# IsseiMori/lajolla_public

Hardware: AMD Instinct MI355X
Metric: Msamples/sec (whole node), cbox 256spp (higher is better)
Workload: dtype f32; 1 GPU; cbox.xml 512x512 @ 256 spp, path integrator (Lambertian + area light, max_depth -1, rr_depth 5); rng=pcg32, one stream per (pixel, sample), seed 0x853c49e6748fea9b, parallelism=1 GPU, collective=none

## Files before the change

### lajolla_public_amd/csrc/device/api_device.hip

```cpp
#include "api_internal.h"

namespace {

void set_device(lj_context *ctx) { HIP_CHECK(hipSetDevice(ctx->device)); }

ljd::DQueue carve_queue(void *base, uint32_t cap) {
    ljd::DQueue q{};
    ljd::Rec4 *p = (ljd::Rec4 *)base;
    auto take = [&]() { ljd::Rec4 *r = p; p += cap; return r; };
    q.ro = take(); q.rd = take(); q.rs = take(); q.rh = take(); q.rw = take(); q.rl = take(); q.rn = take(); q.rg = take();
    return q;
}
size_t queue_bytes(uint32_t cap) { return (size_t)cap * kQueueSlotBytes; }

void ensure_queues(lj_context *ctx, uint32_t cap) {
    if (ctx->queue_capacity >= cap) return;
    cap = (cap + 63u) & ~63u;
    ctx->queue_mem.alloc(queue_bytes(cap));
    ctx->queue_capacity = cap;
}

int *ensure_spill(lj_context *ctx, int levels, uint32_t grid) {
    if (levels <= 0) return nullptr;
    const size_t need = (size_t)levels * grid * 256 * sizeof(int);
// ... 142 lines not shown
    }
    if (plan.rng_mode == LJ_RNG_TILE) { run_tiles(sc, plan, ds, rgb_dev, samples_host, stream); return; }
    const uint64_t max_samples_pass = (uint64_t)1 << 27;
    uint64_t pix_per_pass = std::max<uint64_t>(1, max_samples_pass / (uint64_t)plan.spp);
    pix_per_pass = std::min<uint64_t>(pix_per_pass, n_pix);
    if (sc->flat.integrator == LJ_INTEGRATOR_VOLPATH) {
        const uint64_t pass_samples_max = pix_per_pass * (uint64_t)plan.spp;
        if (ctx->sample_rgb.bytes < pass_samples_max * 12) ctx->sample_rgb.alloc(pass_samples_max * 12);
        if (!ctx->chunk_counter.p) ctx->chunk_counter.alloc(128 * kMaxLanes);
        upload_pixel_list(ctx, plan, stream);
        HIP_CHECK(hipMemsetAsync(ctx->chunk_counter.p, 0, 256, stream));
        HIP_CHECK(hipEventRecord(ctx->ev_begin, stream));
        for (uint64_t p0 = 0; p0 < n_pix; p0 += pix_per_pass) {
            const uint64_t np = std::min<uint64_t>(pix_per_pass, n_pix - p0);
            const uint64_t total = np * (uint64_t)plan.spp;
            ljd::DPass pass{};
            pass.pixel_list = (const uint32_t *)ctx->pixel_list.p + p0; pass.n_pixels = (uint32_t)np; ljd::set_pass_divisors(pass, (uint32_t)plan.spp, (uint32_t)sc->flat.cam.width);
            pass.seed = plan.seed; pass.sample_rgb = (float *)ctx->sample_rgb.p;
            const int grid = (int)std::max<uint64_t>(1, std::min<uint64_t>((total + 255) / 256, (uint64_t)ctx->n_cus * (uint64_t)ljd::volpath_blocks_per_cu(ds)));
            HIP_CHECK(hipMemsetAsync((char *)ctx->chunk_counter.p + 8, 0, 4, stream));
            ljd::launch_volpath(ds, pass, (uint32_t)total, (uint32_t *)ctx->chunk_counter.p, sc->ecfg, sc->scfg.variant,
                                 (sc->feat_kinds & ~7u) == 0u && !sc->feat_textured && !sc->feat_envmap && !sc->feat_sphere_lights,
                                ensure_spill(ctx, sc->ecfg.spill_levels, (uint32_t)grid), grid, stream);
            HIP_CHECK(hipGetLastError());
            st.samples += total; st.wavefront_steps++;
            if (rgb_dev) ljd::launch_resolve(pass, (uint32_t)np, rgb_dev, stream);
            if (samples_host) {
                HIP_CHECK(hipMemcpyAsync(samples_host + p0 * (uint64_t)plan.spp * 3, ctx->sample_rgb.p, total * 12, hipMemcpyDeviceToHost, stream));
                HIP_CHECK(hipStreamSynchronize(stream));
            }
        }
        HIP_CHECK(hipEventRecord(ctx->ev_end, stream));
        HIP_CHECK(hipEventSynchronize(ctx->ev_end));
        float ms = 0; HIP_CHECK(hipEventElapsedTime(&ms, ctx->ev_begin, ctx->ev_end));
        unsigned long long nb = 0;
        HIP_CHECK(hipMemcpy(&nb, ctx->chunk_counter.p, 8, hipMemcpyDeviceToHost));
        st.render_ms = ms; st.bounce_iterations = nb;
        if (getenv("LJ_VOLPATH_STATS")) {
            unsigned long long h[32];
            HIP_CHECK(hipMemcpy(h, ctx->chunk_counter.p, sizeof(h), hipMemcpyDeviceToHost));
            const char *names[8] = {"node iterations", "leaf steps", "closest calls", "tracking (bounce ray)", "tracking (shadow segment)", "shadow segments", "path steps", "-"};
            for (int k = 0; k < 7; k++) fprintf(stderr, "[volpath stats] %-26s wave events %12llu  lanes active %5.1f %%  per sample %.2f\n", names[k], h[2 + 2 * k], h[2 + 2 * k] ? 100.0 * h[3 + 2 * k] / (64.0 * h[2 + 2 * k]) : 0.0, (double)h[3 + 2 * k] / (double)st.samples);
        }
        return;
    }
    const size_t mega_lds = ljd::mega_smem(sc->dscene, sc->scfg);
    const bool mega_off = getenv("LJ_TUNE_MEGA") && atoi(getenv("LJ_TUNE_MEGA")) == 0;
    if (mega_lds > 0 && !mega_off) {
        const uint64_t pass_samples_max = pix_per_pass * (uint64_t)plan.spp;
        if (ctx->sample_rgb.bytes < pass_samples_max * 12) ctx->sample_rgb.alloc(pass_samples_max * 12);
        if (!ctx->mega_state.p) ctx->mega_state.alloc(64);
        upload_pixel_list(ctx, plan, stream);
        HIP_CHECK(hipEventRecord(ctx->ev_begin, stream));
        int per_cu = ljd::mega_blocks_per_cu(sc->scfg);
        if (const char *e = getenv("LJ_TUNE_MEGA_BLOCKS_PER_CU")) per_cu = std::max(1, atoi(e));
        uint32_t grab_max = 768, grab_min = 192;
        bool grab_fixed = false;
        if (const char *e = getenv("LJ_TUNE_MEGA_GRAB")) { grab_max = (uint32_t)std::max(64, atoi(e)) & ~63u; grab_fixed = true; }
        double mega_ms = 0;
        unsigned long long hstats[5] = {};
        for (uint64_t p0 = 0; p0 < n_pix; p0 += pix_per_pass) {
            const uint64_t np = std::min<uint64_t>(pix_per_pass, n_pix - p0);
            const uint64_t total = np * (uint64_t)plan.spp;
            ljd::DPass pass{};
            pass.pixel_list = (const uint32_t *)ctx->pixel_list.p + p0; pass.n_pixels = (uint32_t)np; ljd::set_pass_divisors(pass, (uint32_t)plan.spp, (uint32_t)sc->flat.cam.width);
            pass.seed = plan.seed; pass.sample_rgb = (float *)ctx->sample_rgb.p;
            HIP_CHECK(hipMemsetAsync(ctx->mega_state.p, 0, 64, stream));
            uint32_t grab = grab_max;
            if (!grab_fixed) {
                uint64_t draws = 16;
                if (const char *e = getenv("LJ_TUNE_MEGA_DRAWS")) draws = (uint64_t)std::max(1, atoi(e));
                const uint64_t waves = (uint64_t)ctx->n_cus * per_cu * 4, per_draw = total / (waves * draws);
                grab = (uint32_t)std::min<uint64_t>(grab_max, std::max<uint64_t>(grab_min, per_draw & ~(uint64_t)63));
            }
            const uint64_t pieces = (total + grab - 1) / grab;
            const int grid = (int)std::max<uint64_t>(1, std::min<uint64_t>((uint64_t)ctx->n_cus * per_cu, (pieces + 3) / 4));
            if (timing) HIP_CHECK(hipEventRecord(ctx->ev_k0, stream));
            ljd::launch_mega(ds, pass, sc->scfg, sc->flat.n_spheres > 0, (uint32_t)total, grab, (uint32_t *)ctx->mega_state.p,
                             (unsigned long long *)((char *)ctx->mega_state.p + 8), grid, stream);
            HIP_CHECK(hipGetLastError());
            if (timing) {
                HIP_CHECK(hipEventRecord(ctx->ev_k1, stream)); HIP_CHECK(hipEventSynchronize(ctx->ev_k1));
                float a = 0; HIP_CHECK(hipEventElapsedTime(&a, ctx->ev_k0, ctx->ev_k1)); mega_ms += a;
            }
            st.mega_launches++; st.wavefront_steps++;
            if (rgb_dev) ljd::launch_resolve(pass, (uint32_t)np, rgb_dev, stream);
            unsigned long long *h = ctx->stats_host;
            HIP_CHECK(hipMemcpyAsync(h, (char *)ctx->mega_state.p + 8, 5 * sizeof(unsigned long long), hipMemcpyDeviceToHost, stream));
            if (samples_host) HIP_CHECK(hipMemcpyAsync(samples_host + p0 * (uint64_t)plan.spp * 3, ctx->sample_rgb.p, total * 12, hipMemcpyDeviceToHost, stream));
            HIP_CHECK(hipStreamSynchronize(stream));
            if (h[3] != total)
                throw LjError(LJ_ERR_INTERNAL, "mega launch ended with " + std::to_string(h[3]) + " of " + std::to_string(total) + " samples finished");
            for (int k = 0; k < 5; k++) hstats[k] += h[k];
            st.samples += total;
        }
        HIP_CHECK(hipEventRecord(ctx->ev_end, stream));
        HIP_CHECK(hipEventSynchronize(ctx->ev_end));
        float ms = 0; HIP_CHECK(hipEventElapsedTime(&ms, ctx->ev_begin, ctx->ev_end));
        st.render_ms = ms; st.mega_ms = mega_ms;
        st.bounce_iterations = hstats[0]; st.rays_closest = hstats[1]; st.rays_shadow = hstats[2]; st.path_steps = hstats[4];
        st.mega_bytes = st.samples * 12ull + n_pix * 4ull;
        st.queue_bytes = st.mega_bytes;
        return;
    }
    const uint64_t pass_samples_max = pix_per_pass * (uint64_t)plan.spp;
    uint32_t pool = (uint32_t)std::min<uint64_t>(plan.pool, std::max<uint64_t>(pass_samples_max, 256));
    uint32_t blocks_per_cu = 8;
    if (const char *e = getenv("LJ_TUNE_BLOCKS_PER_CU")) blocks_per_cu = (uint32_t)std::max(1, atoi(e));
    unsigned long long *xstats = nullptr;
    DevBuf xstats_buf;
    if (getenv("LJ_EXTEND_STATS")) { xstats_buf.alloc(64); HIP_CHECK(hipMemsetAsync(xstats_buf.p, 0, 64, stream)); xstats = (unsigned long long *)xstats_buf.p; }
    uint32_t n_lanes = (timing || xstats || pool < (1u << 20)) ? 1u : (pool < (1u << 22) ? 2u : 4u);
    if (sc->scfg.variant >= 4) n_lanes = 1;
    const bool large_tree = ds.n_nodes > sc->ecfg.lds_nodes;
    if (large_tree) n_lanes = 1;
    if (const char *e = getenv("LJ_TUNE_LANES")) n_lanes = (uint32_t)std::min((int)kMaxLanes, std::max(1, atoi(e)));
    uint32_t n_blocks = std::min<uint32_t>(kMaxBlocks, std::max<uint32_t>(n_lanes, std::min<uint32_t>((uint32_t)ctx->n_cus * blocks_per_cu, pool / 256)));
    n_blocks = (n_blocks / n_lanes) * n_lanes;
    const uint32_t lane_blocks = n_blocks / n_lanes;
    uint32_t seg = ((pool + n_blocks - 1) / n_blocks + 255u) & ~255u;
    const uint32_t n_slots = n_blocks * seg, lane_slots = lane_blocks * seg;
    ensure_queues(ctx, n_slots);
    const bool sort_segments = ljd::shade_sorts_segments(sc->scfg);
    if (sort_segments) {
        const uint32_t cap = (n_slots + 63u) & ~63u;
        if (ctx->queue2_capacity < cap) { ctx->queue_mem2.alloc(queue_bytes(cap)); ctx->queue2_capacity = cap; }
        if (ctx->sort_perm.bytes < (size_t)cap * 4) ctx->sort_perm.alloc((size_t)cap * 4);
        if (ctx->sort_keys.bytes < (size_t)cap) ctx->sort_keys.alloc((size_t)cap);
    }
    uint32_t ext_per_cu = n_lanes == 1 ? 8 : (n_lanes == 2 ? 4 : 2);
    if (const char *e = getenv("LJ_TUNE_EXTEND_BLOCKS_PER_CU")) ext_per_cu = (uint32_t)std::max(1, atoi(e));
    const uint32_t lane_chunks = lane_slots / 256u;
    const uint32_t ext_grid = std::max<uint32_t>(1, std::min<uint32_t>((uint32_t)ctx->n_cus * ext_per_cu, (lane_chunks + 3) / 4));
    bool use_tail = !timing && !xstats && !large_tree && ljd::tail_smem(sc->ecfg, sc->scfg) > 0;
    if (const char *e = getenv("LJ_TUNE_TAIL")) use_tail = use_tail && atoi(e) != 0;
    uint64_t tail_num = 1, tail_den = 4;
    if (const char *e = getenv("LJ_TUNE_TAIL_FRAC")) { tail_num = (uint64_t)std::max(1, atoi(e)); tail_den = 16; }
    const uint32_t spill_grid = std::max<uint32_t>(ext_grid, use_tail ? lane_blocks : 0u);
    int *spill_base = ensure_spill(ctx, sc->ecfg.spill_levels, spill_grid * n_lanes);
    if (!ctx->chunk_counter.p) ctx->chunk_counter.alloc(128 * kMaxLanes);
    if (ctx->chunk_list.bytes < (size_t)lane_chunks * 8 * n_lanes) ctx->chunk_list.alloc((size_t)lane_chunks * 8 * n_lanes);
    const ljd::DQueue q_all = carve_queue(ctx->queue_mem.p, ctx->queue_capacity);
    const ljd::DQueue q2_all = sort_segments ? carve_queue(ctx->queue_mem2.p, ctx->queue2_capacity) : q_all;
    struct Lane {
        hipStream_t stream; ljd::DQueue q, q2; uint32_t *sort_perm; uint8_t *sort_keys; ljd::DBlockState *dblocks; ljd::DBlockState *hblocks;
        uint32_t *work; uint32_t *lists[2]; uint32_t parity; int *spill; int *spill_tail; bool done; int batch;
    } lanes[kMaxLanes];
    for (uint32_t l = 0; l < n_lanes; l++) {
        Lane &L = lanes[l];
        L.stream = l == 0 ? stream : ctx->lane_streams[l - 1];
        const size_t o = (size_t)l * lane_slots;
        L.q = q_all; L.q.ro += o; L.q.rd += o; L.q.rs += o; L.q.rh += o; L.q.rw += o; L.q.rl += o; L.q.rn += o; L.q.rg += o;
// ... 86 lines not shown
            }
            if (!any) break;
        }
        uint64_t samples_done = 0, path_steps = 0, shadow_rays = 0;
        for (uint32_t b = 0; b < n_blocks; b++) {
            const ljd::DBlockState &bs = ctx->blocks_host[b];
            samples_done += bs.samples_done; path_steps += bs.path_steps; shadow_rays += bs.rays_shadow;
            st.bounce_iterations += bs.bounce_iterations; st.rays_closest += bs.rays_closest; st.rays_shadow += bs.rays_shadow;
        }
        if (samples_done != total)
            throw LjError(LJ_ERR_INTERNAL, "wavefront loop ended with " + std::to_string(samples_done) + " of " + std::to_string(total) + " samples finished");
        st.samples += total;
        st.path_steps += path_steps;
        st.extend_bytes += path_steps * 48ull + shadow_rays * 16ull;
        st.shade_bytes += path_steps * 224ull + total * 12ull;
        if (rgb_dev) ljd::launch_resolve(pass, (uint32_t)np, rgb_dev, stream);
        if (samples_host) {
            HIP_CHECK(hipMemcpyAsync(samples_host + p0 * (uint64_t)plan.spp * 3, ctx->sample_rgb.p, total * 12, hipMemcpyDeviceToHost, stream));
            HIP_CHECK(hipStreamSynchronize(stream));
        }
    }
    HIP_CHECK(hipEventRecord(ctx->ev_end, stream));
    HIP_CHECK(hipEventSynchronize(ctx->ev_end));
    float ms = 0; HIP_CHECK(hipEventElapsedTime(&ms, ctx->ev_begin, ctx->ev_end));
    st.render_ms = ms; st.extend_ms = extend_ms; st.shade_ms = shade_ms;
    if (xstats) {
        unsigned long long h[8];
        HIP_CHECK(hipMemcpy(h, xstats, 64, hipMemcpyDeviceToHost));
        fprintf(stderr, "[extend stats] rays %llu | outer iters %llu busy lanes %.1f%% | node steps %llu (%.2f/ray) lane use %.1f%% | prim rounds %llu (%.2f tests/ray) lane use %.1f%% | refills %llu\n",
                h[7], h[0], 100.0 * h[1] / (64.0 * h[0]), h[2], (double)h[3] / h[7], 100.0 * h[3] / (64.0 * h[2]), h[4], (double)h[5] / h[7], 100.0 * h[5] / (64.0 * h[4]), h[6]);
    }
    st.queue_bytes = st.extend_bytes + st.shade_bytes;
}

}

extern "C" {

int lj_context_create(int device_id, lj_context **out) {
    return lj::guard([&]() {
        if (!out) throw LjError(LJ_ERR_INVALID_ARG, "lj_context_create: null out");
        *out = nullptr;
        int n = 0;
        hipError_t e = hipGetDeviceCount(&n);
        if (e != hipSuccess || n == 0) throw LjError(LJ_ERR_DEVICE, std::string("no HIP device available (") + hipGetErrorString(e) + "); this library has no CPU path");
        if (device_id < 0 || device_id >= n) throw LjError(LJ_ERR_INVALID_ARG, "device id out of range");
        auto ctx = std::make_unique<lj_context>();
        ctx->device = device_id;
        HIP_CHECK(hipSetDevice(device_id));
        hipDeviceProp_t prop; HIP_CHECK(hipGetDeviceProperties(&prop, device_id));
        if (std::string(prop.gcnArchName).rfind("gfx950", 0) != 0)
            throw LjError(LJ_ERR_DEVICE, std::string("device is ") + prop.gcnArchName + "; this build contains gfx950 code objects only");
        ctx->n_cus = prop.multiProcessorCount;
        HIP_CHECK(hipStreamCreateWithFlags(&ctx->stream, hipStreamNonBlocking));
        for (auto &ls : ctx->lane_streams) HIP_CHECK(hipStreamCreateWithFlags(&ls, hipStreamNonBlocking));
        HIP_CHECK(hipEventCreateWithFlags(&ctx->ev_fork, hipEventDisableTiming)); HIP_CHECK(hipEventCreateWithFlags(&ctx->ev_join, hipEventDisableTiming));
        HIP_CHECK(hipEventCreateWithFlags(&ctx->ev_caller, hipEventDisableTiming));
        ctx->blocks.alloc(sizeof(ljd::DBlockState) * kMaxBlocks);
        HIP_CHECK(hipHostMalloc((void **)&ctx->blocks_host, sizeof(ljd::DBlockState) * kMaxBlocks, hipHostMallocDefault));
        HIP_CHECK(hipHostMalloc((void **)&ctx->stats_host, 64, hipHostMallocDefault));
        HIP_CHECK(hipEventCreate(&ctx->ev_begin)); HIP_CHECK(hipEventCreate(&ctx->ev_end));
        HIP_CHECK(hipEventCreate(&ctx->ev_k0)); HIP_CHECK(hipEventCreate(&ctx->ev_k1));
        *out = ctx.release();
    });
}

void lj_context_destroy(lj_context *ctx) {
    if (!ctx) return;
    if (ctx->live_scenes > 0) { ctx->doomed = true; return; }
    (void)hipSetDevice(ctx->device);
    if (ctx->stream) { (void)hipStreamSynchronize(ctx->stream); (void)hipStreamDestroy(ctx->stream); }
    for (auto &ls : ctx->lane_streams) if (ls) { (void)hipStreamSynchronize(ls); (void)hipStreamDestroy(ls); }
    if (ctx->ev_fork) (void)hipEventDestroy(ctx->ev_fork);
    if (ctx->ev_join) (void)hipEventDestroy(ctx->ev_join);
    if (ctx->ev_caller) (void)hipEventDestroy(ctx->ev_caller);
    if (ctx->blocks_host) (void)hipHostFree(ctx->blocks_host);
    if (ctx->stats_host) (void)hipHostFree(ctx->stats_host);
    for (hipEvent_t e : {ctx->ev_begin, ctx->ev_end, ctx->ev_k0, ctx->ev_k1}) if (e) (void)hipEventDestroy(e);
    delete ctx;
}

int lj_scene_upload(lj_context *ctx, const LjSceneDesc *desc, lj_scene **out) {
    return lj::guard([&]() {
        if (!ctx || !desc || !out) throw LjError(LJ_ERR_INVALID_ARG, "lj_scene_upload: null argument");
        *out = nullptr;
        set_device(ctx);
        auto sc = std::make_unique<lj_scene>();
        sc->ctx = ctx;
        sc->flat = lj::flatten_scene(*desc);
        lj::FlatScene &F = sc->flat;
        hipStream_t s = ctx->stream;
        upload(sc->nodes, F.nodes, s);
        int node8_stride = (int)sizeof(ljd::DNode8);
        if (const char *e = getenv("LJ_TUNE_NODE8_STRIDE")) node8_stride = atoi(e) >= 128 ? 128 : 80;
        std::vector<unsigned char> nodes8_padded;
        if (node8_stride == (int)sizeof(ljd::DNode8)) upload(sc->nodes8, F.nodes8, s);
        else {
            nodes8_padded.assign(F.nodes8.size() * (size_t)node8_stride, 0);
            for (size_t i = 0; i < F.nodes8.size(); i++) memcpy(&nodes8_padded[i * (size_t)node8_stride], &F.nodes8[i], sizeof(ljd::DNode8));
            upload(sc->nodes8, nodes8_padded, s);
        }
        upload(sc->leaf_prims, F.leaf_prims, s); upload(sc->prims, F.prims, s); upload(sc->spheres, F.spheres, s);
        upload(sc->materials, F.materials, s); upload(sc->lights, F.lights, s); upload(sc->light_cdf, F.light_cdf, s);
        upload(sc->light_tris, F.light_tris, s); upload(sc->light_tri_cdf, F.light_tri_cdf, s);
        upload(sc->images3, F.images3, s); upload(sc->images1, F.images1, s); upload(sc->texels, F.texels, s); upload(sc->env_tables, F.env_tables, s);
        upload(sc->media, F.media, s); upload(sc->volume_data, F.volume_data, s); upload(sc->shape_media, F.shape_media, s);
// ... 137 lines not shown
```

### lajolla_public_amd/csrc/device/api_internal.h

```cpp
#pragma once
#include <hip/hip_runtime.h>
#include "../host/api_common.h"
#include "../host/flatten.h"
#include "dtypes.h"
#include "dconfig.h"
#include <algorithm>
#include <cstdlib>
#include <cstring>
#include <memory>
#include <string>
#include <vector>

namespace ljd {
ShadeConfig shade_config(size_t n_prims, size_t n_materials, size_t n_lights, size_t n_light_tris, size_t n_light_tri_cdf, size_t n_images3, size_t n_images1, size_t n_env_marg);
int shade_variant(uint32_t kinds, bool textured, bool envmap, bool sphere_lights);
ExtendConfig extend_config(int n_nodes, int n_prims, int bvh_depth, int n_spheres, int n_nodes8, int bvh8_depth, bool open_scene);
int max_stack_depth();
void launch_extend(const DScene &sc, const DQueue &q, const DBlockState *blocks, uint32_t grid, uint32_t seg, uint32_t *work, const uint32_t *chunk_list, uint32_t parity, const ExtendConfig &cfg, int *spill, unsigned long long *stats, hipStream_t s);
bool shade_sorts_segments(const ShadeConfig &cfg);
void launch_shade(const DScene &sc, const DPass &pass, const DQueue &q, const DQueue &qo, uint32_t *sort_perm, uint8_t *sort_keys, DBlockState *blocks, uint32_t n_blocks, uint32_t seg, const ShadeConfig &cfg, uint32_t *work, uint32_t *chunk_list, uint32_t parity, uint32_t extend_waves, hipStream_t s);
void launch_resolve(const DPass &pass, uint32_t n_pixels, float *rgb, hipStream_t s);
size_t tail_smem(const ExtendConfig &ecfg, const ShadeConfig &scfg);
void launch_tail(const DScene &sc, const DPass &pass, const DQueue &q, DBlockState *blocks, uint32_t n_blocks, uint32_t seg, const ExtendConfig &ecfg, const ShadeConfig &scfg, int *spill, hipStream_t s);
void launch_aux(const DScene &sc, const uint32_t *pixel_list, uint32_t n_pixels, int integrator, float *rgb, const ExtendConfig &cfg, int *spill, int grid, hipStream_t s);
void launch_volpath(const DScene &sc, const DPass &pass, uint32_t n_samples, uint32_t *counters, const ExtendConfig &cfg, int shade_variant, bool plain, int *spill, int grid, hipStream_t s);
int volpath_blocks_per_cu(const DScene &sc);
void launch_trace_rays(const DScene &sc, const void *rays, long long n, void *hits, unsigned char *occ, const ExtendConfig &cfg, int *spill, int grid, hipStream_t s);
size_t mega_smem(const DScene &sc, const ShadeConfig &scfg);
int mega_blocks_per_cu(const ShadeConfig &scfg);
void launch_mega(const DScene &sc, const DPass &pass, const ShadeConfig &scfg, bool spheres, uint32_t n_samples, uint32_t grab, uint32_t *sample_counter, unsigned long long *stats, int grid, hipStream_t s);
void launch_trace_rays_scan(const DScene &sc, const void *rays, long long n, void *hits, unsigned char *occ, int grid, hipStream_t s);
size_t tile_cursor_bytes(bool vol);
void launch_tile_init(bool vol, void *cursors, const uint32_t *tiles, uint32_t n_tiles, uint64_t seed, hipStream_t s);
int tile_grid(uint32_t n_tiles, uint32_t lanes);
void launch_tile(bool vol, const DScene &sc, const DTileJob &job, void *cursors, uint32_t lanes, uint32_t budget, uint32_t *alive, const ExtendConfig &cfg, int *spill, hipStream_t s);
void tile_cursor_stats(bool vol, const void *cursors_host, uint32_t n, unsigned long long out[5]);
}

using lj::LjError;

#define HIP_CHECK(expr) do { hipError_t _e = (expr); if (_e != hipSuccess) \
    throw LjError(LJ_ERR_DEVICE, std::string(#expr) + " failed: " + hipGetErrorString(_e)); } while (0)

struct DevBuf {
    void *p = nullptr; size_t bytes = 0;
    void alloc(size_t n) { release(); if (n) { HIP_CHECK(hipMalloc(&p, n)); bytes = n; } }
    void release() { if (p) { (void)hipFree(p); p = nullptr; bytes = 0; } }
    ~DevBuf() { release(); }
    DevBuf() = default; DevBuf(const DevBuf &) = delete; DevBuf &operator=(const DevBuf &) = delete;
};

template <typename T> inline void upload(DevBuf &b, const std::vector<T> &v, hipStream_t s) {
    b.alloc(((std::max<size_t>(v.size(), 1) * sizeof(T)) + 31) & ~(size_t)15);
    if (!v.empty()) HIP_CHECK(hipMemcpyAsync(b.p, v.data(), v.size() * sizeof(T), hipMemcpyHostToDevice, s));
}

static constexpr size_t kQueueSlotBytes = 128;
static constexpr uint32_t kMaxBlocks = 8192;

static constexpr uint32_t kMaxLanes = 8;
struct lj_context {
    int device = 0;
    int live_scenes = 0; bool doomed = false;
    hipStream_t stream = nullptr;
    hipStream_t lane_streams[kMaxLanes - 1] = {};
    hipEvent_t ev_fork = nullptr, ev_join = nullptr, ev_caller = nullptr;
    int n_cus = 256;
    DevBuf queue_mem; uint32_t queue_capacity = 0;
    DevBuf queue_mem2, sort_perm, sort_keys; uint32_t queue2_capacity = 0;
    DevBuf chunk_counter, chunk_list;
    DevBuf spill;
    DevBuf blocks, sample_rgb, pixel_list, frame;
    uint64_t pixel_list_key = 0;
    DevBuf tile_cursors, tile_list, tile_samples;
    DevBuf mega_state;
    ljd::DBlockState *blocks_host = nullptr;
    unsigned long long *stats_host = nullptr;
    hipEvent_t ev_begin = nullptr, ev_end = nullptr, ev_k0 = nullptr, ev_k1 = nullptr;
};

struct lj_scene {
    lj_context *ctx = nullptr;
    lj::FlatScene flat;
    DevBuf nodes, nodes8, leaf_prims, prims, spheres, materials, lights, light_cdf, light_tris, light_tri_cdf, images3, images1, texels, env_tables;
    DevBuf media, volume_data, shape_media, scan_leaves;
    ljd::DScene dscene{};
    ljd::ExtendConfig ecfg{};
    ljd::ShadeConfig scfg{};
    uint32_t feat_kinds = 0; bool feat_textured = false, feat_envmap = false, feat_sphere_lights = false;
    std::shared_ptr<const std::vector<uint32_t>> plan_pixels; uint64_t plan_pixels_key = 0;
    std::vector<int64_t> shape_first_gprim;
    LjStats stats{};
};
```

### lajolla_public_amd/csrc/device/mega.hip

```cpp
#include "dstage.h"
#include "dtrace.h"
#include "dconfig.h"

namespace ljd {

#define LJ_CONST __attribute__((address_space(4)))

constexpr uint32_t kItemCap = 512;
constexpr uint32_t kWaveScanBytes = 64 * 48 + 64 * 8 + 64 * 4 + kItemCap * 2;

struct ScanCtx {
    const LJ_CONST float *boxes;
    int n_used;
    const LJ_LDS int *leaf_tab;
    const LJ_LDS v4f *lprims; int prim_stride;
    const DSphere *spheres;
    LJ_LDS v4f *rays;
    LJ_LDS unsigned long long *keys;
    LJ_LDS uint32_t *occl;
    LJ_LDS uint16_t *items;
};

__device__ __forceinline__ uint32_t lane_id() { return __builtin_amdgcn_mbcnt_hi(~0u, __builtin_amdgcn_mbcnt_lo(~0u, 0u)); }

struct ScanRay { float ix, iy, iz, ox, oy, oz; };
__device__ __forceinline__ ScanRay scan_ray(f3 org, f3 dir) {
    const float tiny = 1e-18f;
    const float dx = fabsf(dir.x) < tiny ? copysignf(tiny, dir.x) : dir.x, dy = fabsf(dir.y) < tiny ? copysignf(tiny, dir.y) : dir.y,
                dz = fabsf(dir.z) < tiny ? copysignf(tiny, dir.z) : dir.z;
    ScanRay r;
    r.ix = __builtin_amdgcn_rcpf(dx); r.iy = __builtin_amdgcn_rcpf(dy); r.iz = __builtin_amdgcn_rcpf(dz);
    r.ox = org.x * r.ix; r.oy = org.y * r.iy; r.oz = org.z * r.iz;
    return r;
}
template <bool FAR>
__device__ __forceinline__ float scan_box(const float (&b)[6], const ScanRay &r, float tnear, float tfar) {
    const float ax = __builtin_fmaf(b[0], r.ix, -r.ox), bx = __builtin_fmaf(b[3], r.ix, -r.ox);
    const float ay = __builtin_fmaf(b[1], r.iy, -r.oy), by = __builtin_fmaf(b[4], r.iy, -r.oy);
    const float az = __builtin_fmaf(b[2], r.iz, -r.oz), bz = __builtin_fmaf(b[5], r.iz, -r.oz);
    const float te = fmaxf(fmaxf(fminf(ax, bx), fminf(ay, by)), fmaxf(fminf(az, bz), tnear));
    float tx = fminf(fminf(fmaxf(ax, bx), fmaxf(ay, by)), fmaxf(az, bz));
    if (FAR) tx = fminf(tx, tfar);
    return __builtin_fmaf(tx, -1.0000005f, te);
}
__device__ __forceinline__ uint32_t shift_in_sign(uint32_t mask, float d) { return __builtin_amdgcn_alignbit(mask, f2u(d), 31u); }

template <bool E, bool S>
__device__ __forceinline__ void scan_leaf_boxes(const ScanCtx &sx, const ScanRay &re, float tnear_e, const ScanRay &rs, float tnear_s, float tfar_s, uint32_t &me, uint32_t &ms) {
    const int n = sx.n_used;
    int k = 0;
    for (; k + 4 <= n; k += 4) {
        float b[4][6];
#pragma unroll
        for (int c = 0; c < 4; c++)
#pragma unroll
            for (int j = 0; j < 6; j++) b[c][j] = sx.boxes[(k + c) * 8 + j];
#pragma unroll
        for (int c = 0; c < 4; c++) {
            if (E) me = shift_in_sign(me, scan_box<false>(b[c], re, tnear_e, INFINITY));
            if (S) ms = shift_in_sign(ms, scan_box<true>(b[c], rs, tnear_s, tfar_s));
        }
    }
    for (; k < n; k++) {
        float b[6];
#pragma unroll
        for (int j = 0; j < 6; j++) b[j] = sx.boxes[k * 8 + j];
        if (E) me = shift_in_sign(me, scan_box<false>(b, re, tnear_e, INFINITY));
        if (S) ms = shift_in_sign(ms, scan_box<true>(b, rs, tnear_s, tfar_s));
    }
}
__device__ __forceinline__ void scan_leaf_boxes2(const ScanCtx &sx, f3 org, f3 dir_e, float tnear_e, f3 dir_s, float tnear_s, float tfar_s, bool any_e, bool any_s,
                                                 uint32_t &me, uint32_t &ms) {
    const ScanRay re = scan_ray(org, dir_e), rs = scan_ray(org, dir_s);
    tnear_e = fmaxf(tnear_e, 0.0f); tnear_s = fmaxf(tnear_s, 0.0f);
    me = 0u; ms = 0u;
    if (any_e && any_s) scan_leaf_boxes<true, true>(sx, re, tnear_e, rs, tnear_s, tfar_s, me, ms);
    else if (any_e) scan_leaf_boxes<true, false>(sx, re, tnear_e, rs, tnear_s, tfar_s, me, ms);
    else if (any_s) scan_leaf_boxes<false, true>(sx, re, tnear_e, rs, tnear_s, tfar_s, me, ms);
}

template <bool SPHERES>
__device__ __forceinline__ void scan_trace(const ScanCtx &sx, bool has_e, bool has_s, f3 org, f3 dir_e, float tnear_e, f3 dir_s, float tnear_s, float tfar_s,
                                           float &ht, float &hu, float &hv, int &gprim_out, bool &occluded) {
#pragma clang fp contract(off)
    const uint32_t lane = lane_id();
    uint32_t me = 0, ms = 0;
    scan_leaf_boxes2(sx, org, dir_e, tnear_e, dir_s, tnear_s, tfar_s, __ballot(has_e) != 0ull, __ballot(has_s) != 0ull, me, ms);
    me = has_e ? me : 0u; ms = has_s ? ms : 0u;
    v4f r0, r1, r2;
    r0.x = org.x; r0.y = org.y; r0.z = org.z; r0.w = tfar_s;
    r1.x = dir_e.x; r1.y = dir_e.y; r1.z = dir_e.z; r1.w = tnear_e;
    r2.x = dir_s.x; r2.y = dir_s.y; r2.z = dir_s.z; r2.w = tnear_s;
    sx.rays[lane * 3] = r0; sx.rays[lane * 3 + 1] = r1; sx.rays[lane * 3 + 2] = r2;
    sx.keys[lane] = ~0ull; sx.occl[lane] = 0u;
    for (;;) {
        uint32_t n_items = 0;
        for (;;) {
            const bool has = (ms | me) != 0u;
            const unsigned long long b = __ballot(has);
            if (b == 0ull || n_items + 64u > kItemCap) break;
            if (has) {
                uint32_t leaf, kind;
                if (ms) { leaf = (uint32_t)(sx.n_used - 1) - (uint32_t)__builtin_ctz(ms); ms &= ms - 1u; kind = 1u; }
                else { leaf = (uint32_t)(sx.n_used - 1) - (uint32_t)__builtin_ctz(me); me &= me - 1u; kind = 0u; }
                const uint32_t idx = n_items + __builtin_amdgcn_mbcnt_hi((uint32_t)(b >> 32), __builtin_amdgcn_mbcnt_lo((uint32_t)b, 0u));
                sx.items[idx] = (uint16_t)(lane | (leaf << 6) | (kind << 11));
            }
            n_items += (uint32_t)__popcll(b);
        }
        if (n_items == 0u) break;
        __builtin_amdgcn_fence(__ATOMIC_RELEASE, "wavefront"); __builtin_amdgcn_wave_barrier();
        for (uint32_t r = 0; r < n_items; r += 64u) {
            if (r + lane < n_items) {
                const uint32_t it = sx.items[r + lane];
                const uint32_t src = it & 63u, leaf = (it >> 6) & 31u, kind = it >> 11;
                const v4f o4 = sx.rays[src * 3], d4 = sx.rays[src * 3 + 1 + kind];
                RayF ray;
                ray.ox = o4.x; ray.oy = o4.y; ray.oz = o4.z; ray.dx = d4.x; ray.dy = d4.y; ray.dz = d4.z;
                ray.tnear = d4.w; ray.tfar = kind ? o4.w : INFINITY;
                const int first = sx.leaf_tab[2 * leaf], cnt = sx.leaf_tab[2 * leaf + 1];
                for (int p = 0; p < cnt; p++) {
                    const int pi = first + p, S = sx.prim_stride;
                    const v4f p0 = sx.lprims[pi], p1 = sx.lprims[S + pi], p2 = sx.lprims[2 * S + pi];
                    const int gprim = __float_as_int(p0.w);
                    bool hit; float t;
                    if (!SPHERES || __float_as_int(p1.w) == 0) {
                        const float v0[3] = {p0.x, p0.y, p0.z}, v1[3] = {p1.x, p1.y, p1.z}, v2[3] = {p2.x, p2.y, p2.z};
                        float U, V, Ssum;
                        hit = tri_test_raw(ray, ray.tfar, v0, v1, v2, t, U, V, Ssum);
                    } else {
                        double td = 0.0;
                        hit = sphere_test(ray, sx.spheres[__float_as_int(p2.w)], td);
                        t = (float)td;
                    }
                    if (hit) {
                        if (kind) sx.occl[src] = 1u;
                        else (void)__hip_atomic_fetch_min(&sx.keys[src], ((unsigned long long)f2u(t) << 32) | (unsigned long long)(((uint32_t)gprim << 16) | (uint32_t)pi), __ATOMIC_RELAXED, __HIP_MEMORY_SCOPE_WAVEFRONT);
                    }
                }
            }
        }
        __builtin_amdgcn_fence(__ATOMIC_RELEASE, "wavefront"); __builtin_amdgcn_wave_barrier();
        if (__ballot((ms | me) != 0u) == 0ull) break;
    }
    const unsigned long long key = sx.keys[lane];
    const uint32_t low = (uint32_t)key;
    occluded = sx.occl[lane] != 0u;
    gprim_out = -1; ht = 0.0f; hu = 0.0f; hv = 0.0f;
    if (has_e && low != 0xffffffffu) {
        const int pi = (int)(low & 0xffffu), S = sx.prim_stride;
        gprim_out = (int)(low >> 16);
        ht = u2f((uint32_t)(key >> 32));
        const v4f p0 = sx.lprims[pi], p1 = sx.lprims[S + pi], p2 = sx.lprims[2 * S + pi];
        if (!SPHERES || __float_as_int(p1.w) == 0) {
            RayF ray;
            ray.ox = org.x; ray.oy = org.y; ray.oz = org.z; ray.dx = dir_e.x; ray.dy = dir_e.y; ray.dz = dir_e.z; ray.tnear = tnear_e; ray.tfar = INFINITY;
            const float v0[3] = {p0.x, p0.y, p0.z}, v1[3] = {p1.x, p1.y, p1.z}, v2[3] = {p2.x, p2.y, p2.z};
            float t, U, V, Ssum;
            (void)tri_test_raw(ray, INFINITY, v0, v1, v2, t, U, V, Ssum);
            const float rS = div_ieee(1.0f, Ssum);
            hu = U * rS; hv = V * rS;
        }
    }
}

__device__ __forceinline__ f3 add_rounded(f3 a, f3 b) {
#pragma clang fp contract(off)
    return mk3(a.x + b.x, a.y + b.y, a.z + b.z);
}

__device__ __forceinline__ void opaque(float &x) { asm volatile("" : "+v"(x)); }
__device__ __forceinline__ void opaque(f3 &v) { opaque(v.x); opaque(v.y); opaque(v.z); }
__device__ __forceinline__ void opaque_state(PathState &ps) {
    opaque(ps.org); opaque(ps.dir); opaque(ps.ht); opaque(ps.hu); opaque(ps.hv); opaque(ps.sdir); opaque(ps.stfar);
    opaque(ps.W); opaque(ps.rr); opaque(ps.p2); opaque(ps.rad); opaque(ps.nee); opaque(ps.eta_scale); opaque(ps.spread);
}

__device__ __forceinline__ ScanCtx stage_scan(const DScene &sc, uint32_t at) {
    ScanCtx sx;
    char *base = (char *)lj_smem + at;
    LJ_LDS int *lt = (LJ_LDS int *)base;
    for (int i = threadIdx.x; i < sc.n_scan_leaves; i += kBlock) { lt[2 * i] = sc.scan_leaves[i].first; lt[2 * i + 1] = sc.scan_leaves[i].count; }
    const uint32_t lt_bytes = ((uint32_t)sc.n_scan_leaves * 8u + 15u) & ~15u;
    LJ_LDS v4f *lp = (LJ_LDS v4f *)(base + lt_bytes);
    const v4f *src = reinterpret_cast<const v4f *>(sc.leaf_prims);
    for (int i = threadIdx.x; i < sc.n_prims * 3; i += kBlock) lp[(i % 3) * sc.n_prims + (i / 3)] = src[i];
    char *wave = base + lt_bytes + (uint32_t)sc.n_prims * 48u + (threadIdx.x >> 6) * kWaveScanBytes;
    sx.boxes = (const LJ_CONST float *)(uintptr_t)sc.scan_leaves; sx.n_used = sc.n_scan_used;
    sx.leaf_tab = lt; sx.lprims = lp; sx.prim_stride = sc.n_prims; sx.spheres = sc.spheres;
    sx.rays = (LJ_LDS v4f *)wave; sx.keys = (LJ_LDS unsigned long long *)(wave + 64 * 48); sx.occl = (LJ_LDS uint32_t *)(wave + 64 * 48 + 64 * 8);
    sx.items = (LJ_LDS uint16_t *)(wave + 64 * 48 + 64 * 8 + 64 * 4);
    return sx;
}
size_t scan_smem(int n_scan_leaves, int n_prims) { return (((size_t)n_scan_leaves * 8 + 15) & ~(size_t)15) + (size_t)n_prims * 48 + 4 * (size_t)kWaveScanBytes; }

#ifndef LJ_MEGA_OCC
#define LJ_MEGA_OCC 5
#endif
template <class Ft> struct MegaOccupancy { static constexpr int waves = 3; };
template <> struct MegaOccupancy<FeatLambert> { static constexpr int waves = LJ_MEGA_OCC; };
#ifndef LJ_MEGA_OCC_PLASTIC
#define LJ_MEGA_OCC_PLASTIC 4
#endif
template <> struct MegaOccupancy<FeatPlastic> { static constexpr int waves = LJ_MEGA_OCC_PLASTIC; };

template <class Ft, bool SPHERES>
__global__ void __launch_bounds__(kBlock, MegaOccupancy<Ft>::waves) k_mega(DScene sc, DPass pass, ShadeStage stg, uint32_t scan_at, uint32_t n_samples, uint32_t grab,
                                                              uint32_t *sample_counter, unsigned long long *stats) {
    stage_shade_tables<2>(sc, stg, 0u);
    const ScanCtx sx = stage_scan(sc, scan_at);
    __syncthreads();
    const uint32_t lane = lane_id();
    ShadeCounters cnt; cnt.bounces = cnt.closest = cnt.shadow = cnt.done = 0;
    uint32_t steps = 0;
    bool live = false, exhausted = false;
    uint32_t w_next = 0, w_end = 0;
    PathState ps;
    ps.flags = 0u; ps.stfar = 0.0f; ps.sample = 0u;
    for (;;) {
        opaque_state(ps);
        if (live) {
            steps++;
            if (!shade_path<Ft>(sc, pass, ps, cnt)) {
                float *o = pass.sample_rgb + 3ull * ps.sample;
                o[0] = ps.rad.x; o[1] = ps.rad.y; o[2] = ps.rad.z;
                cnt.done++; live = false;
            }
        }
        const unsigned long long dead = __ballot(!live);
        if (dead != 0ull && !exhausted) {
            if (w_next == w_end) {
                uint32_t b = 0;
                if (lane == 0u) b = atomicAdd(sample_counter, grab);
                b = (uint32_t)__builtin_amdgcn_readfirstlane((int)b);
                if (b >= n_samples) exhausted = true;
                else { w_next = b; w_end = (n_samples - b < grab) ? n_samples : b + grab; }
            }
            if (!exhausted) {
                const uint32_t left = w_end - w_next, n_dead = (uint32_t)__popcll(dead);
                const uint32_t rank = __builtin_amdgcn_mbcnt_hi((uint32_t)(dead >> 32), __builtin_amdgcn_mbcnt_lo((uint32_t)dead, 0u));
                if (!live && rank < left) { generate_path(sc, pass, w_next + rank, ps); live = true; }
                w_next += n_dead < left ? n_dead : left;
            }
        }
        if (__ballot(live) == 0ull) { if (exhausted) break; else continue; }
        opaque_state(ps);
        const bool has_e = live && !(ps.flags & PF_NO_EXT), has_s = live && ps.stfar > 0.0f;
        float ht, hu, hv; int gprim; bool occluded;
        scan_trace<SPHERES>(sx, has_e, has_s, ps.org, ps.dir, (ps.flags & 0xffffu) == 2u ? 0.0f : sc.eps, ps.sdir, sc.eps, ps.stfar, ht, hu, hv, gprim, occluded);
        if (live) {
            if (has_s && !occluded) ps.rad = add_rounded(ps.rad, ps.nee);
            ps.ht = ht; ps.hu = hu; ps.hv = hv; ps.hcode = gprim + 1;
            if (ps.flags & PF_NO_EXT) {
                float *o = pass.sample_rgb + 3ull * ps.sample;
                o[0] = ps.rad.x; o[1] = ps.rad.y; o[2] = ps.rad.z;
                cnt.done++; live = false;
            }
        }
    }
    const uint32_t b = wave_sum(cnt.bounces), cl = wave_sum(cnt.closest), sh = wave_sum(cnt.shadow), dn = wave_sum(cnt.done), sp = wave_sum(steps);
    if (lane == 0u) {
        atomicAdd(&stats[0], (unsigned long long)b); atomicAdd(&stats[1], (unsigned long long)cl); atomicAdd(&stats[2], (unsigned long long)sh);
        atomicAdd(&stats[3], (unsigned long long)dn); atomicAdd(&stats[4], (unsigned long long)sp);
    }
}

struct RayIO { float org[3]; float tnear; float dir[3]; float tfar; };
struct HitIO { float t, u, v; int32_t shape_id, prim_id; };
__global__ void __launch_bounds__(kBlock) k_trace_rays_scan(DScene sc, const RayIO *rays, long long n, HitIO *hits, unsigned char *occ) {
    const ScanCtx sx = stage_scan(sc, 0u);
    __syncthreads();
    const long long stride = (long long)gridDim.x * kBlock;
    for (long long i0 = (long long)blockIdx.x * kBlock; i0 < n; i0 += stride) {
        const long long i = i0 + threadIdx.x;
        const bool act = i < n;
        f3 org = mk3(0, 0, 0), dir = mk3(0, 0, 1); float tn = 0.0f, tf = 0.0f;
        if (act) { org = ld3(rays[i].org); dir = ld3(rays[i].dir); tn = rays[i].tnear; tf = rays[i].tfar; }
        float ht, hu, hv; int gprim; bool occluded;
        if (occ) {
            scan_trace<true>(sx, false, act, org, dir, 0.0f, dir, tn, tf, ht, hu, hv, gprim, occluded);
            if (act) occ[i] = occluded ? 1 : 0;
        } else {
            scan_trace<true>(sx, act, false, org, dir, tn, dir, 0.0f, 0.0f, ht, hu, hv, gprim, occluded);
            if (act) {
                HitIO o; o.t = 0; o.u = 0; o.v = 0; o.shape_id = -1; o.prim_id = -1;
                if (gprim >= 0 && ht <= tf) { const DPrimShade &ps = sc.prims[gprim]; o.t = ht; o.u = hu; o.v = hv; o.shape_id = ps.shape_id; o.prim_id = ps.prim_id; }
                hits[i] = o;
            }
        }
    }
}


size_t mega_smem(const DScene &sc, const ShadeConfig &scfg) {
    if (sc.n_scan_leaves <= 0 || !scfg.stage_prims || scfg.smem == 0) return 0;
    const size_t at = (scfg.smem + 15) & ~(size_t)15, total = at + scan_smem(sc.n_scan_leaves, sc.n_prims);
    return total <= 64 * 1024 ? total : 0;
}

int mega_blocks_per_cu(const ShadeConfig &scfg) {
    int waves = 3;
    with_shade_variant(scfg.variant, [&](auto ft) { waves = MegaOccupancy<decltype(ft)>::waves; });
    return waves;
}

void launch_mega(const DScene &sc, const DPass &pass, const ShadeConfig &scfg, bool spheres, uint32_t n_samples, uint32_t grab, uint32_t *sample_counter,
                 unsigned long long *stats, int grid, hipStream_t s) {
    const ShadeStage st = make_shade_stage(scfg);
    const uint32_t at = (uint32_t)((scfg.smem + 15) & ~(size_t)15);
    const size_t smem = mega_smem(sc, scfg);
    with_shade_variant(scfg.variant, [&](auto ft) {
        using Ft = decltype(ft);
        if (spheres) hipLaunchKernelGGL((k_mega<Ft, true>), dim3(grid), dim3(kBlock), smem, s, sc, pass, st, at, n_samples, grab, sample_counter, stats);
        else hipLaunchKernelGGL((k_mega<Ft, false>), dim3(grid), dim3(kBlock), smem, s, sc, pass, st, at, n_samples, grab, sample_counter, stats);
    });
}

void launch_trace_rays_scan(const DScene &sc, const void *rays, long long n, void *hits, unsigned char *occ, int grid, hipStream_t s) {
    hipLaunchKernelGGL(k_trace_rays_scan, dim3(grid), dim3(kBlock), scan_smem(sc.n_scan_leaves, sc.n_prims), s, sc, (const RayIO *)rays, n, (HitIO *)hits, occ);
}

}
```

Measured before the change: 5478 Msamples/s.

## Flatten leaf primitive tests into a per-wave item pool and cap mega grid by LDS

The mega-kernel scan now expands each lane's pending leaves into one item per primitive in a wave-local LDS list. The whole wave then tests those (ray, primitive) pairs 64 at a time, instead of each lane looping over its own leaf's primitives with the others idle. This targets lane divergence when leaves hold different primitive counts. It costs extra ballots, LDS writes and reloads of the ray per item. Separately, blocks per CU for the mega grid is now capped by how many workgroups fit in the device's LDS, and optional stats counters are added.

```diff
diff --git a/lajolla_public_amd/csrc/device/api_device.hip b/lajolla_public_amd/csrc/device/api_device.hip
--- a/lajolla_public_amd/csrc/device/api_device.hip
+++ b/lajolla_public_amd/csrc/device/api_device.hip
@@ -218,7 +218,7 @@
         if (!ctx->mega_state.p) ctx->mega_state.alloc(64);
         upload_pixel_list(ctx, plan, stream);
         HIP_CHECK(hipEventRecord(ctx->ev_begin, stream));
-        int per_cu = ljd::mega_blocks_per_cu(sc->scfg);
+        int per_cu = ljd::mega_blocks_per_cu(sc->scfg, mega_lds, ctx->lds_per_cu);
         if (const char *e = getenv("LJ_TUNE_MEGA_BLOCKS_PER_CU")) per_cu = std::max(1, atoi(e));
         uint32_t grab_max = 768, grab_min = 192;
         bool grab_fixed = false;
@@ -264,6 +264,13 @@
         HIP_CHECK(hipEventSynchronize(ctx->ev_end));
         float ms = 0; HIP_CHECK(hipEventElapsedTime(&ms, ctx->ev_begin, ctx->ev_end));
         st.render_ms = ms; st.mega_ms = mega_ms;
+        if (getenv("LJ_MEGA_INFO")) {
+            fprintf(stderr, "[mega] LDS %zu B per workgroup, %zu B per CU: %d workgroups per CU\n", mega_lds, ctx->lds_per_cu, per_cu);
+            unsigned long long ps[4];
+            if (ljd::mega_pool_stats(ps))
+                fprintf(stderr, "[mega] primitive tests: %llu wave issues, lanes live %.1f %% | sample generation: %llu wave issues for %llu samples (%.1f %% of lanes), %.3f issues per path-step of a wave\n",
+                        ps[0], ps[0] ? 100.0 * ps[1] / (64.0 * ps[0]) : 0.0, ps[2], ps[3], ps[2] ? 100.0 * ps[3] / (64.0 * ps[2]) : 0.0, hstats[4] ? ps[2] * 64.0 / hstats[4] : 0.0);
+        }
         st.bounce_iterations = hstats[0]; st.rays_closest = hstats[1]; st.rays_shadow = hstats[2]; st.path_steps = hstats[4];
         st.mega_bytes = st.samples * 12ull + n_pix * 4ull;
         st.queue_bytes = st.mega_bytes;
@@ -456,6 +463,7 @@
         if (std::string(prop.gcnArchName).rfind("gfx950", 0) != 0)
             throw LjError(LJ_ERR_DEVICE, std::string("device is ") + prop.gcnArchName + "; this build contains gfx950 code objects only");
         ctx->n_cus = prop.multiProcessorCount;
+        ctx->lds_per_cu = std::max<size_t>(ctx->lds_per_cu, prop.maxSharedMemoryPerMultiProcessor);
         HIP_CHECK(hipStreamCreateWithFlags(&ctx->stream, hipStreamNonBlocking));
         for (auto &ls : ctx->lane_streams) HIP_CHECK(hipStreamCreateWithFlags(&ls, hipStreamNonBlocking));
         HIP_CHECK(hipEventCreateWithFlags(&ctx->ev_fork, hipEventDisableTiming)); HIP_CHECK(hipEventCreateWithFlags(&ctx->ev_join, hipEventDisableTiming));
diff --git a/lajolla_public_amd/csrc/device/api_internal.h b/lajolla_public_amd/csrc/device/api_internal.h
--- a/lajolla_public_amd/csrc/device/api_internal.h
+++ b/lajolla_public_amd/csrc/device/api_internal.h
@@ -27,7 +27,8 @@
 int volpath_blocks_per_cu(const DScene &sc);
 void launch_trace_rays(const DScene &sc, const void *rays, long long n, void *hits, unsigned char *occ, const ExtendConfig &cfg, int *spill, int grid, hipStream_t s);
 size_t mega_smem(const DScene &sc, const ShadeConfig &scfg);
-int mega_blocks_per_cu(const ShadeConfig &scfg);
+int mega_blocks_per_cu(const ShadeConfig &scfg, size_t smem, size_t lds_per_cu);
+bool mega_pool_stats(unsigned long long out[4]);
 void launch_mega(const DScene &sc, const DPass &pass, const ShadeConfig &scfg, bool spheres, uint32_t n_samples, uint32_t grab, uint32_t *sample_counter, unsigned long long *stats, int grid, hipStream_t s);
 void launch_trace_rays_scan(const DScene &sc, const void *rays, long long n, void *hits, unsigned char *occ, int grid, hipStream_t s);
 size_t tile_cursor_bytes(bool vol);
@@ -66,6 +67,7 @@
     hipStream_t lane_streams[kMaxLanes - 1] = {};
     hipEvent_t ev_fork = nullptr, ev_join = nullptr, ev_caller = nullptr;
     int n_cus = 256;
+    size_t lds_per_cu = 160 * 1024;
     DevBuf queue_mem; uint32_t queue_capacity = 0;
     DevBuf queue_mem2, sort_perm, sort_keys; uint32_t queue2_capacity = 0;
     DevBuf chunk_counter, chunk_list;
diff --git a/lajolla_public_amd/csrc/device/mega.hip b/lajolla_public_amd/csrc/device/mega.hip
--- a/lajolla_public_amd/csrc/device/mega.hip
+++ b/lajolla_public_amd/csrc/device/mega.hip
@@ -6,8 +6,21 @@
 
 #define LJ_CONST __attribute__((address_space(4)))
 
+#ifndef LJ_MEGA_PRIM_ITEMS
+#define LJ_MEGA_PRIM_ITEMS 1
+#endif
+
 constexpr uint32_t kItemCap = 512;
+static_assert(kItemCap >= 64 * 8, "a pass must admit one round whatever its leaves hold: 64 lanes x 8 primitives (flatten.cpp)");
 constexpr uint32_t kWaveScanBytes = 64 * 48 + 64 * 8 + 64 * 4 + kItemCap * 2;
+
+#ifdef LJ_MEGA_POOL_STATS
+__device__ unsigned long long g_pool_stats[4];
+#define LJ_POOL_STAT(k) do { const unsigned long long m_ = __ballot(true); \
+    if (lane_id() == (uint32_t)__builtin_ctzll(m_)) { atomicAdd(&g_pool_stats[k], 1ull); atomicAdd(&g_pool_stats[(k) + 1], (unsigned long long)__popcll(m_)); } } while (0)
+#else
+#define LJ_POOL_STAT(k) do { } while (0)
+#endif
 
 struct ScanCtx {
     const LJ_CONST float *boxes;
@@ -77,6 +90,28 @@
     if (any_e && any_s) scan_leaf_boxes<true, true>(sx, re, tnear_e, rs, tnear_s, tfar_s, me, ms);
     else if (any_e) scan_leaf_boxes<true, false>(sx, re, tnear_e, rs, tnear_s, tfar_s, me, ms);
     else if (any_s) scan_leaf_boxes<false, true>(sx, re, tnear_e, rs, tnear_s, tfar_s, me, ms);
+}
+
+template <bool SPHERES>
+__device__ __forceinline__ void test_prim(const ScanCtx &sx, const RayF &ray, uint32_t src, uint32_t kind, int pi) {
+#pragma clang fp contract(off)
+    const int S = sx.prim_stride;
+    const v4f p0 = sx.lprims[pi], p1 = sx.lprims[S + pi], p2 = sx.lprims[2 * S + pi];
+    const int gprim = __float_as_int(p0.w);
+    bool hit; float t;
+    if (!SPHERES || __float_as_int(p1.w) == 0) {
+        const float v0[3] = {p0.x, p0.y, p0.z}, v1[3] = {p1.x, p1.y, p1.z}, v2[3] = {p2.x, p2.y, p2.z};
+        float U, V, Ssum;
+        hit = tri_test_raw(ray, ray.tfar, v0, v1, v2, t, U, V, Ssum);
+    } else {
+        double td = 0.0;
+        hit = sphere_test(ray, sx.spheres[__float_as_int(p2.w)], td);
+        t = (float)td;
+    }
+    if (hit) {
+        if (kind) sx.occl[src] = 1u;
+        else (void)__hip_atomic_fetch_min(&sx.keys[src], ((unsigned long long)f2u(t) << 32) | (unsigned long long)(((uint32_t)gprim << 16) | (uint32_t)pi), __ATOMIC_RELAXED, __HIP_MEMORY_SCOPE_WAVEFRONT);
+    }
 }
 
 template <bool SPHERES>
@@ -95,6 +130,46 @@
     sx.keys[lane] = ~0ull; sx.occl[lane] = 0u;
     for (;;) {
         uint32_t n_items = 0;
+#if LJ_MEGA_PRIM_ITEMS
+        for (;;) {
+            const bool has = (ms | me) != 0u;
+            const unsigned long long b = __ballot(has);
+            if (b == 0ull) break;
+            uint32_t first = 0u, c1 = 0u;
+            const uint32_t kind = ms ? 1u : 0u;
+            if (has) {
+                const uint32_t leaf = (uint32_t)(sx.n_used - 1) - (uint32_t)__builtin_ctz(ms ? ms : me);
+                first = (uint32_t)sx.leaf_tab[2 * leaf]; c1 = (uint32_t)sx.leaf_tab[2 * leaf + 1] - 1u;
+            }
+            const unsigned long long b0 = __ballot((c1 & 1u) != 0u), b1 = __ballot((c1 & 2u) != 0u), b2 = __ballot((c1 & 4u) != 0u);
+            const uint32_t total = (uint32_t)__popcll(b) + (uint32_t)__popcll(b0) + 2u * (uint32_t)__popcll(b1) + 4u * (uint32_t)__popcll(b2);
+            if (n_items + total > kItemCap) break;
+            if (has) {
+                if (kind) ms &= ms - 1u; else me &= me - 1u;
+                const uint32_t at = n_items + __builtin_amdgcn_mbcnt_hi((uint32_t)(b >> 32), __builtin_amdgcn_mbcnt_lo((uint32_t)b, 0u))
+                                  + __builtin_amdgcn_mbcnt_hi((uint32_t)(b0 >> 32), __builtin_amdgcn_mbcnt_lo((uint32_t)b0, 0u))
+                                  + 2u * __builtin_amdgcn_mbcnt_hi((uint32_t)(b1 >> 32), __builtin_amdgcn_mbcnt_lo((uint32_t)b1, 0u))
+                                  + 4u * __builtin_amdgcn_mbcnt_hi((uint32_t)(b2 >> 32), __builtin_amdgcn_mbcnt_lo((uint32_t)b2, 0u));
+                const uint32_t it0 = lane | (first << 6) | (kind << 14);
+                for (uint32_t j = 0; j <= (c1 & 7u); j++) sx.items[at + j] = (uint16_t)(it0 + (j << 6));
+            }
+            n_items += total;
+        }
+        if (n_items == 0u) break;
+        __builtin_amdgcn_fence(__ATOMIC_RELEASE, "wavefront"); __builtin_amdgcn_wave_barrier();
+        for (uint32_t r = 0; r < n_items; r += 64u) {
+            if (r + lane < n_items) {
+                LJ_POOL_STAT(0);
+                const uint32_t it = sx.items[r + lane];
+                const uint32_t src = it & 63u, kind = it >> 14;
+                const v4f o4 = sx.rays[src * 3], d4 = sx.rays[src * 3 + 1 + kind];
+                RayF ray;
+                ray.ox = o4.x; ray.oy = o4.y; ray.oz = o4.z; ray.dx = d4.x; ray.dy = d4.y; ray.dz = d4.z;
+                ray.tnear = d4.w; ray.tfar = kind ? o4.w : INFINITY;
+                test_prim<SPHERES>(sx, ray, src, kind, (int)((it >> 6) & 255u));
+            }
+        }
+#else
         for (;;) {
             const bool has = (ms | me) != 0u;
             const unsigned long long b = __ballot(has);
@@ -119,27 +194,10 @@
                 ray.ox = o4.x; ray.oy = o4.y; ray.oz = o4.z; ray.dx = d4.x; ray.dy = d4.y; ray.dz = d4.z;
                 ray.tnear = d4.w; ray.tfar = kind ? o4.w : INFINITY;
                 const int first = sx.leaf_tab[2 * leaf], cnt = sx.leaf_tab[2 * leaf + 1];
-                for (int p = 0; p < cnt; p++) {
-                    const int pi = first + p, S = sx.prim_stride;
-                    const v4f p0 = sx.lprims[pi], p1 = sx.lprims[S + pi], p2 = sx.lprims[2 * S + pi];
-                    const int gprim = __float_as_int(p0.w);
-                    bool hit; float t;
-                    if (!SPHERES || __float_as_int(p1.w) == 0) {
-                        const float v0[3] = {p0.x, p0.y, p0.z}, v1[3] = {p1.x, p1.y, p1.z}, v2[3] = {p2.x, p2.y, p2.z};
-                        float U, V, Ssum;
-                        hit = tri_test_raw(ray, ray.tfar, v0, v1, v2, t, U, V, Ssum);
-                    } else {
-                        double td = 0.0;
-                        hit = sphere_test(ray, sx.spheres[__float_as_int(p2.w)], td);
-                        t = (float)td;
-                    }
-                    if (hit) {
-                        if (kind) sx.occl[src] = 1u;
-                        else (void)__hip_atomic_fetch_min(&sx.keys[src], ((unsigned long long)f2u(t) << 32) | (unsigned long long)(((uint32_t)gprim << 16) | (uint32_t)pi), __ATOMIC_RELAXED, __HIP_MEMORY_SCOPE_WAVEFRONT);
-                    }
-                }
-            }
-        }
+                for (int p = 0; p < cnt; p++) { LJ_POOL_STAT(0); test_prim<SPHERES>(sx, ray, src, kind, first + p); }
+            }
+        }
+#endif
         __builtin_amdgcn_fence(__ATOMIC_RELEASE, "wavefront"); __builtin_amdgcn_wave_barrier();
         if (__ballot((ms | me) != 0u) == 0ull) break;
     }
@@ -176,6 +234,7 @@
     opaque(ps.W); opaque(ps.rr); opaque(ps.p2); opaque(ps.rad); opaque(ps.nee); opaque(ps.eta_scale); opaque(ps.spread);
 }
 
+__host__ __device__ inline uint32_t scan_bytes(int n_scan_leaves, int n_prims) { return (((uint32_t)n_scan_leaves * 8u + 15u) & ~15u) + (uint32_t)n_prims * 48u + 4u * kWaveScanBytes; }
 __device__ __forceinline__ ScanCtx stage_scan(const DScene &sc, uint32_t at) {
     ScanCtx sx;
     char *base = (char *)lj_smem + at;
@@ -192,7 +251,7 @@
     sx.items = (LJ_LDS uint16_t *)(wave + 64 * 48 + 64 * 8 + 64 * 4);
     return sx;
 }
-size_t scan_smem(int n_scan_leaves, int n_prims) { return (((size_t)n_scan_leaves * 8 + 15) & ~(size_t)15) + (size_t)n_prims * 48 + 4 * (size_t)kWaveScanBytes; }
+size_t scan_smem(int n_scan_leaves, int n_prims) { return scan_bytes(n_scan_leaves, n_prims); }
 
 #ifndef LJ_MEGA_OCC
 #define LJ_MEGA_OCC 5
@@ -239,7 +298,7 @@
             if (!exhausted) {
                 const uint32_t left = w_end - w_next, n_dead = (uint32_t)__popcll(dead);
                 const uint32_t rank = __builtin_amdgcn_mbcnt_hi((uint32_t)(dead >> 32), __builtin_amdgcn_mbcnt_lo((uint32_t)dead, 0u));
-                if (!live && rank < left) { generate_path(sc, pass, w_next + rank, ps); live = true; }
+                if (!live && rank < left) { LJ_POOL_STAT(2); generate_path(sc, pass, w_next + rank, ps); live = true; }
                 w_next += n_dead < left ? n_dead : left;
             }
         }
@@ -298,10 +357,22 @@
     return total <= 64 * 1024 ? total : 0;
 }
 
-int mega_blocks_per_cu(const ShadeConfig &scfg) {
+int mega_blocks_per_cu(const ShadeConfig &scfg, size_t smem, size_t lds_per_cu) {
     int waves = 3;
     with_shade_variant(scfg.variant, [&](auto ft) { waves = MegaOccupancy<decltype(ft)>::waves; });
-    return waves;
+    const size_t granted = (smem + 1279) / 1280 * 1280;
+    const int by_lds = granted ? (int)(lds_per_cu / granted) : waves;
+    return std::max(1, std::min(waves, by_lds));
+}
+
+bool mega_pool_stats(unsigned long long out[4]) {
+#ifdef LJ_MEGA_POOL_STATS
+    const unsigned long long zero[4] = {};
+    if (hipMemcpyFromSymbol(out, HIP_SYMBOL(g_pool_stats), sizeof(zero)) != hipSuccess) return false;
+    return hipMemcpyToSymbol(HIP_SYMBOL(g_pool_stats), zero, sizeof(zero)) == hipSuccess;
+#else
+    (void)out; return false;
+#endif
 }
 
 void launch_mega(const DScene &sc, const DPass &pass, const ShadeConfig &scfg, bool spheres, uint32_t n_samples, uint32_t grab, uint32_t *sample_counter,
```

New measurement: 4898 Msamples/s. 0.894x the previous value.
